# pixeru/bpm_analysis

Hardware: AMD Instinct MI355X
Metric: audio-samples/sec (filter+envelope+peaks), 1024x60s@44.1kHz batch, 1 & 8 GPU (higher is better)
Workload: dtype f64; 1 GPU; 1024 x 60 s 44100 Hz mono int16 recordings per GPU, native mode (filter+envelope+noise floor+raw peaks); mode=native, parallelism=file-sharded x1, batch_pipeline=False

## Files before the change

bpm_analysis_amd/_native.py:

```python
from __future__ import annotations

import ctypes
import os

_HERE = os.path.dirname(os.path.abspath(__file__))
LIB_PATH = os.environ.get("BPMX_LIB") or os.path.join(_HERE, "libbpmx.so")

ABI_VERSION = 2

DT_U8, DT_I16, DT_I32, DT_F32, DT_F64 = 0, 1, 2, 3, 4
MODE_REFERENCE, MODE_NATIVE = 0, 1
STAGE_ENVELOPE, STAGE_FLOOR, STAGE_PEAKS, STAGE_ALL = 1, 2, 4, 7
F_STATIC_FLOOR, F_DRAFT_FLOOR, F_NAN_FLOOR, F_TOO_SHORT, F_BAD_WINDOW = 1, 2, 4, 8, 16
F_TROUGH_TIE, F_PEAK_TIE = 32, 64
F_TROUGH_ORDERED, F_PEAK_ORDERED = 128, 256
OPT_ROLLQ_MERGE = 1
OPT_NATIVE_F64 = 2
OPT_HILBERT_ROCFFT = 4
OPT_DRAFT_FULL = 8
OPT_ROLLQ_NOPRUNE = 16
OPT_DRAFT_GLOBAL_RANK = 32
OPT_ROLLQ_GLOBAL = 64
OPT_NATIVE_DMA = 128
OPT_PEAKS_GLOBAL = 256
OPT_HILBERT_R2C = 512
OPT_REF_SERIAL_MEAN = 1024
OPT_STATS = 2048
OPT_HILBERT_BLUESTEIN = 4096
OPT_REF_NOSPLIT = 8192
STAT_RAW_TROUGHS, STAT_UNDECIDED, STAT_FULL_DRAFT, NSTATS = 0, 1, 2, 8
OK, E_ARG, E_HIP, E_LIMIT, E_NODEV = 0, -1, -2, -3, -4

EXPORTS = ["bpmx_abi_version", "bpmx_last_error", "bpmx_create", "bpmx_destroy", "bpmx_decimated_length",
           "bpmx_run", "bpmx_run_ordered", "bpmx_synth", "bpmx_synth_host", "bpmx_profile", "bpmx_profile_read", "bpmx_profile_only",
           "bpmx_stats", "bpmx_set_pipeline"]


class Params(ctypes.Structure):
    _fields_ = [("mode", ctypes.c_int32), ("stages", ctypes.c_int32), ("dtype", ctypes.c_int32),
                ("channels", ctypes.c_int32), ("fs", ctypes.c_int32), ("ds", ctypes.c_int32),
                ("sr", ctypes.c_int32), ("env_window", ctypes.c_int32), ("distance", ctypes.c_int32),
                ("noise_window", ctypes.c_int32), ("min_periods", ctypes.c_int32), ("options", ctypes.c_int32),
                ("trough_prom_q", ctypes.c_double), ("peak_prom_q", ctypes.c_double),
                ("noise_floor_q", ctypes.c_double), ("fallback_q", ctypes.c_double),
                ("reject_mult", ctypes.c_double),
                ("ba_b", ctypes.c_double * 5), ("ba_a", ctypes.c_double * 5), ("ba_zi", ctypes.c_double * 4),
                ("sos", ctypes.c_double * 12), ("sos_zi", ctypes.c_double * 4)]


class Batch(ctypes.Structure):
    _fields_ = [("n_files", ctypes.c_int32), ("reserved", ctypes.c_int32), ("pcm", ctypes.c_void_p),
                ("frame_offsets", ctypes.POINTER(ctypes.c_int64))]


class Out(ctypes.Structure):
    _fields_ = [("env", ctypes.c_void_p), ("floor", ctypes.c_void_p), ("y", ctypes.c_void_p),
                ("troughs", ctypes.c_void_p), ("peaks", ctypes.c_void_p), ("n_troughs", ctypes.c_void_p),
                ("n_peaks", ctypes.c_void_p), ("flags", ctypes.c_void_p), ("n_raw_troughs", ctypes.c_void_p)]


class PeakOrder(ctypes.Structure):
    _fields_ = [("cand", ctypes.c_void_p * 2), ("n_cand", ctypes.c_void_p * 2),
                ("rank", ctypes.c_void_p * 2), ("use_rank", ctypes.c_void_p * 2)]


class BpmxError(RuntimeError):

    def __init__(self, msg: str = "", code: int = None):
        super().__init__(msg)
        self.code = code

    @property
    def per_file(self) -> bool:
        return self.code in (E_ARG, E_LIMIT)


class BpmxArgError(BpmxError, ValueError):
    """BPMX_E_ARG: an argument the reference's own calls reject with ValueError
    (scipy find_peaks' distance check, pandas' rolling-window checks); the
    message is the library's, which repeats the reference-side wording."""


_lib = None
# ... 51 lines not shown
```

bpm_analysis_amd/csrc/bpmx_api.hip:

```cpp
#include <hip/hip_runtime.h>

#include <algorithm>
#include <climits>
#include <cstdio>
#include <cstring>
#include <cstdlib>
#include <map>
#include <mutex>
#include <string>
#include <vector>

#include "bpmx_common.h"
#include "bpmx_kernels.h"
#include "bpmx_ctx.h"
#include "bpmx_native.h"
#include "bpmx_fpscan.h"
#include "bpmx_synth.h"

#include <rocprofiler-sdk-roctx/roctx.h>

using namespace bpmx;

namespace bpmx {
thread_local std::string g_err;
// ... 622 lines not shown
            FIND_PEAKS(a, "troughs");
        }
        if (bad_window)
            LAUNCH(ctx, s, "k_flag_window", k_flag_window, dim3((F + 255) / 256), dim3(256), 0, s, F, d_run1,
                   (int32_t *)O->flags);
        const bool floor_wm = !(P->options & (BPMX_OPT_ROLLQ_MERGE | BPMX_OPT_ROLLQ_GLOBAL | BPMX_OPT_ROLLQ_NOPRUNE)) &&
                              maxnd <= WM_MMAX;
        if (noise_lazy && !floor_wm) {
            QuantArgs a;
            a.env = O->env; a.doff = d_doff; a.active = d_active; a.n_files = F; a.qv = qv; a.skip_le = QR_MAX;
            a.n_levels = 1; a.q[0] = P->noise_floor_q; a.slot[0] = 1 << Q_NOISE;
            a.skip = d_run1; a.stats = 0;
            LAUNCH(ctx, s, "k_quantile_reg", k_quantile_reg, dim3(F), dim3(QR_T), 0, s, a, bs);
        }
        const int64_t W = bad_window ? P->min_periods : P->noise_window;
        const int cap = (int)((W + RQ_T - 1 + 63) / 64 * 64);
        const size_t lds = rollq_lds_bytes(RQ_T, cap);
        const bool use_wm = !(P->options & (BPMX_OPT_ROLLQ_MERGE | BPMX_OPT_ROLLQ_GLOBAL));
        const bool need_merge = !use_wm || maxnd > WM_MMAX;
        const bool merge_g = need_merge && (cap > 32 * RQ_T || W + RQ_T >= 65000 || (P->options & BPMX_OPT_ROLLQ_GLOBAL));
        const int64_t gcap = (std::min<int64_t>(W + RQ_T, maxnd + 64) + 63) / 64 * 64;
        const size_t lds_g = rollq_g_lds_bytes(RQ_T, gcap);
        if (merge_g && lds_g > 160 * 1024)
            return fail(BPMX_E_LIMIT, "noise window and recording both longer than " +
                                          std::to_string((160 * 1024 - 16384) / 4 * 64) + " samples");
        uint16_t *wm_pos = use_wm ? (uint16_t *)ctx->buf("wm_pos", (size_t)sumnd * 2, &rc) : nullptr;
        int32_t *wm_full = use_wm ? (int32_t *)ctx->buf("wm_full", (size_t)F * 4, &rc) : nullptr;
        if (rc != BPMX_OK) return rc;
        const int64_t wm_n = std::min<int64_t>(maxnd, WM_MMAX);
        const size_t wm_lds_p = wm_layout(wm_n, true).total, wm_lds = wm_layout(wm_n, false).total;
        const int64_t wm_c = (WM_MMAX - W + 1) / 64 * 64;
        const bool wm_chunks = use_wm && maxnd > WM_MMAX && !(P->options & BPMX_OPT_ROLLQ_NOPRUNE) && wm_c >= 2048;
        const int64_t wm_nch = wm_chunks ? (maxnd + wm_c - 1) / wm_c : 1;
        int32_t *wm_fail = wm_chunks ? (int32_t *)ctx->buf("wm_fail", (size_t)F * 4, &rc) : nullptr;
        uint16_t *wm_pos_ch = wm_chunks ? (uint16_t *)ctx->buf("wm_pos_ch", (size_t)F * wm_nch * WM_PMAX * 2, &rc) : nullptr;
        if (rc != BPMX_OK) return rc;
        if (wm_nch > 65535) return fail(BPMX_E_LIMIT, "recording too long for the chunked rolling quantile");
        const dim3 g2((unsigned)std::min<int64_t>((maxnd + 255) / 256, std::max<int64_t>(8, 2048 / F)), F);
        auto interp = [&](const int32_t *run, const int64_t *tr, const int32_t *ntr, int64_t skip_gt) -> int {
            InterpArgs a;
            a.env = O->env; a.doff = d_doff; a.troughs = tr; a.ntr = ntr; a.run = run; a.n_files = F;
            a.dense = dense; a.skip_n = use_wm ? WM_MMAX : -1; a.skip_gt = skip_gt;
            const dim3 gi = maxnd <= WM_MMAX && use_wm ? dim3(2, (unsigned)F) : g2;
            LAUNCH(ctx, s, "k_interp", k_interp, gi, dim3(256), 0, s, a);
            return BPMX_OK;
        };
        auto rollq = [&](const int32_t *run, const int64_t *tr, const int32_t *ntr, double *outp,
                         int32_t *allnan, const double *tv) -> int {
            RollqArgs a;
            a.dense = dense; a.doff = d_doff; a.troughs = tr; a.tv = tv; a.run = run; a.n_files = F;
            a.env = O->env; a.ntr = ntr;
            a.window = (int32_t)W; a.min_periods = P->min_periods; a.cap = cap; a.q = P->noise_floor_q;
            a.out = outp; a.allnan = allnan; a.wm_max = use_wm ? WM_MMAX : 0;
            a.wm_chunk = 0; a.wm_fail = wm_fail; a.wm_pos_ch = wm_pos_ch;
            int rq_rc = BPMX_OK;
            int32_t *vfl = need_merge ? (int32_t *)ctx->buf("rollq_valid", (size_t)F * 8, &rq_rc) : nullptr;
            if (rq_rc != BPMX_OK) return rq_rc;
            a.vfirst = vfl;
            a.vlast = vfl ? vfl + F : nullptr;
            if (need_merge) {
                HIP_TRY(hipMemsetAsync(a.vfirst, 0x7F, (size_t)F * 4, s));
                HIP_TRY(hipMemsetAsync(a.vlast, 0xFF, (size_t)F * 4, s));
            }
            if (wm_chunks) {
                HIP_TRY(hipMemsetAsync(wm_fail, 0, (size_t)F * 4, s));
                a.wm_chunk = (int32_t)wm_c;
            }
            if (need_merge && (rq_rc = interp(run, tr, ntr, wm_chunks ? WM_MMAX : INT64_MAX)) != BPMX_OK) return rq_rc;
            if (use_wm) {
                wm_lds_attr(ctx->device);
                if (!(P->options & BPMX_OPT_ROLLQ_NOPRUNE))
                    LAUNCH(ctx, s, "k_rollq_wm", k_rollq_wm_t<true>, dim3(F, (unsigned)wm_nch), dim3(WM_T),
                           std::max(wm_lds_p, wm_lds), s, a, wm_pos, wm_full);
                else
                    LAUNCH(ctx, s, "k_rollq_wm[full]", k_rollq_wm_t<false>, dim3(F), dim3(WM_T), wm_lds, s, a, wm_pos,
                           wm_full);
            }
            if (!need_merge) return BPMX_OK;
            RollqArgs fill = a;
            if (wm_chunks) {
                a.run = wm_fail;
                if ((rq_rc = interp(wm_fail, tr, ntr, INT64_MAX)) != BPMX_OK) return rq_rc;
            }
            a.chunk = 8192;
            while (a.chunk > 1024 && (int64_t)F * ((maxnd + a.chunk - 1) / a.chunk) < 1024) a.chunk >>= 1;
            if (merge_g) a.chunk = std::max<int64_t>(a.chunk, (W + RQ_T - 1) / RQ_T * RQ_T);
            const int64_t nch = (maxnd + a.chunk - 1) / a.chunk;
            if (nch > 65535) return fail(BPMX_E_LIMIT, "recording too long for the chunked rolling quantile");
            const dim3 gq((unsigned)F, (unsigned)nch);
            if (merge_g) {
                a.gcap = gcap;
                a.gv = (double *)ctx->buf("rollq_gv", (size_t)F * nch * 2 * gcap * 8, &rq_rc);
                a.gp = (int32_t *)ctx->buf("rollq_gp", (size_t)F * nch * 2 * gcap * 4, &rq_rc);
                if (rq_rc != BPMX_OK) return rq_rc;
                (void)hipFuncSetAttribute((const void *)k_rolling_quantile_g<RQ_T>,
                                          hipFuncAttributeMaxDynamicSharedMemorySize, (int)lds_g);
                LAUNCH(ctx, s, "k_rolling_quantile", (k_rolling_quantile_g<RQ_T>), gq, dim3(RQ_T), lds_g, s, a);
            } else if (cap <= 16 * RQ_T) {
                (void)hipFuncSetAttribute((const void *)k_rolling_quantile<RQ_T, 16>,
                                          hipFuncAttributeMaxDynamicSharedMemorySize, (int)lds);
                LAUNCH(ctx, s, "k_rolling_quantile", (k_rolling_quantile<RQ_T, 16>), gq, dim3(RQ_T), lds, s, a);
            } else {
                (void)hipFuncSetAttribute((const void *)k_rolling_quantile<RQ_T, 32>,
                                          hipFuncAttributeMaxDynamicSharedMemorySize, (int)lds);
                LAUNCH(ctx, s, "k_rolling_quantile", (k_rolling_quantile<RQ_T, 32>), gq, dim3(RQ_T), lds, s, a);
            }
            LAUNCH(ctx, s, "k_rollq_fill", k_rollq_fill, dim3(4, (unsigned)F), dim3(256), 0, s, fill);
            return BPMX_OK;
        };
        uint8_t *tdec = nullptr;
        int32_t *d_exact = d_run1, *d_runfb = nullptr;
        if (bounds) {
            tdec = (uint8_t *)ctx->buf("trough_dec", (size_t)sumnd, &rc);
            if (rc != BPMX_OK) return rc;
            d_exact = draft_masks;
            d_runfb = draft_masks + F;
            DraftBoundArgs a;
            a.env = O->env; a.doff = d_doff; a.raw = rawt; a.rawv = rawv; a.nraw = d_nraw; a.run = d_run1;
            a.n_files = F;
            a.window = (int32_t)W; a.min_periods = P->min_periods; a.q = P->noise_floor_q; a.mult = P->reject_mult;
            a.dec = tdec; a.exact = d_exact;
            a.local_m = (P->options & BPMX_OPT_DRAFT_GLOBAL_RANK) ? INT_MAX : DB_LOCAL_M;
            a.stats = d_stats;
            if (rc != BPMX_OK) return rc;
            const int64_t trmax = maxnd / std::max<int64_t>(1, P->distance) + 1;
            const unsigned gy = (unsigned)std::max<int64_t>(1, (trmax + DB_T - 1) / DB_T);
            a.vfl = draft_vfl;
            a.nund = draft_vfl + 2 * F;
            LAUNCH(ctx, s, "k_draft_bounds", k_draft_bounds, dim3(F, gy), dim3(DB_T), 0, s, a);
#ifndef BPMX_DP_GY
#define BPMX_DP_GY 4
#endif
            const unsigned gp = (unsigned)std::max<int64_t>(1, std::min<int64_t>(BPMX_DP_GY, (trmax + DP_CHUNK - 1) / DP_CHUNK));
            LAUNCH(ctx, s, "k_draft_points", k_draft_points<1>, dim3(F, gp), dim3(DB_T), 0, s, a);
            LAUNCH(ctx, s, "k_draft_points[wide]", k_draft_points<4>, dim3(F, gp), dim3(DB_T), 0, s, a);
        }
        SanitizeArgs sa;
        sa.env = O->env; sa.draft = draft; sa.doff = d_doff; sa.active = d_active; sa.raw = rawt; sa.nraw = d_nraw;
        sa.rawv = rawv; sa.outv = trv;
        sa.n_files = F; sa.mult = P->reject_mult; sa.out = O->troughs; sa.nout = O->n_troughs; sa.flags = O->flags;
        sa.run2 = d_run2; sa.dec = tdec; sa.exact = d_exact; sa.run_fb = d_runfb;
        if (floor_wm) {
            FloorWmArgs a;
            a.rq.dense = dense; a.rq.doff = d_doff; a.rq.n_files = F; a.rq.env = O->env;
            a.rq.window = (int32_t)W; a.rq.min_periods = P->min_periods; a.rq.cap = cap; a.rq.q = P->noise_floor_q;
            a.rq.wm_max = WM_MMAX; a.rq.wm_chunk = 0; a.rq.wm_fail = nullptr; a.rq.wm_pos_ch = nullptr;
            a.rq.vfirst = a.rq.vlast = nullptr; a.rq.chunk = 0; a.rq.gv = nullptr; a.rq.gp = nullptr; a.rq.gcap = 0;
            a.rq.troughs = nullptr; a.rq.tv = nullptr; a.rq.ntr = nullptr; a.rq.run = nullptr; a.rq.out = nullptr;
            a.rq.allnan = nullptr;
#ifdef BPMX_STAMPS
            a.rq.stamps = nullptr;
#endif
            sa.run2 = nullptr; sa.run_fb = nullptr;
            a.sa = sa;
            a.exact = d_exact;
            a.qv = qv;
            a.qn = QuantArgs{};
            if (noise_lazy) {
                a.qn.env = O->env; a.qn.doff = d_doff; a.qn.active = d_active; a.qn.n_files = F; a.qn.qv = qv;
                a.qn.skip_le = QR_MAX; a.qn.n_levels = 1; a.qn.q[0] = P->noise_floor_q; a.qn.slot[0] = 1 << Q_NOISE;
                a.qn.skip = nullptr; a.qn.stats = 0;
            }
            a.floor = O->floor; a.draft = draft; a.an_draft = d_an1; a.an_final = d_an2; a.full = wm_full;
            if ((rc = rollq(d_exact, rawt, d_nraw, draft, d_an1, rawv)) != BPMX_OK) return rc;
            wm_lds_attr(ctx->device);
            LAUNCH(ctx, s, "k_floor_wm", k_floor_wm, dim3(F), dim3(WM_T), std::max(wm_lds_p, wm_lds), s, a);
        }
        if (!floor_wm && (rc = rollq(d_exact, rawt, d_nraw, draft, d_an1, rawv)) != BPMX_OK) return rc;
        if (!floor_wm) {
            SanitizeArgs a;
            a.env = O->env; a.draft = draft; a.doff = d_doff; a.active = d_active; a.raw = rawt; a.nraw = d_nraw;
            a.rawv = rawv; a.outv = trv;
            a.n_files = F; a.mult = P->reject_mult; a.out = O->troughs; a.nout = O->n_troughs; a.flags = O->flags;
            a.run2 = d_run2; a.dec = tdec; a.exact = d_exact; a.run_fb = d_runfb;
            LAUNCH(ctx, s, "k_sanitize", k_sanitize, dim3(F), dim3(256), 0, s, a);
        }
        if (!floor_wm && bounds && (rc = rollq(d_runfb, rawt, d_nraw, draft, d_an1, rawv)) != BPMX_OK) return rc;
        if (!floor_wm && (rc = rollq(d_run2, O->troughs, O->n_troughs, O->floor, d_an2, trv)) != BPMX_OK) return rc;
        if (!floor_wm) {
            FinalArgs a;
            a.draft = draft; a.doff = d_doff; a.active = d_active; a.qv = qv; a.allnan_draft = d_an1;
            a.allnan_final = d_an2; a.n_files = F; a.floor = O->floor; a.flags = O->flags;
#ifndef BPMX_FF_WIDE
            const dim3 gf(maxnd > 65536 ? g2.x : 1u, (unsigned)F);
#else
            const dim3 gf = g2;
#endif
            LAUNCH(ctx, s, "k_floor_final", k_floor_final, gf, dim3(256), 0, s, a);
        }
    }

    if (do_peaks) {
        StageRange range("bpmx:peaks");
        PeakArgs a;
        a.env = O->env; a.height = O->floor; a.doff = d_doff; a.boff = d_boff; a.active = d_active;
        a.bmax = bmax; a.bmin = bmin; a.qv = qv; a.qslot = Q_PEAK; a.n_files = F; a.distance = P->distance;
        a.sign = 1.0; a.cand = cand; a.state = state; a.out = O->peaks; a.nout = O->n_peaks;
        a.run_out = nullptr; a.run_min = 0; a.tie_bit = BPMX_F_PEAK_TIE;
        a.scan_ok = fp_scan; a.scan_cnt = fp_scan + F;
        set_order(a, 1);
        FIND_PEAKS(a, "peaks");
    }
// ... 161 lines not shown
```

bpm_analysis_amd/csrc/bpmx_kernels.h:

```cpp
#ifndef BPMX_KERNELS_H
#define BPMX_KERNELS_H

#include "bpmx_common.h"

namespace bpmx {

enum { Q_TROUGH = 0, Q_PEAK = 1, Q_NOISE = 2, Q_FALLBACK = 3, Q_SLOTS = 4 };

struct InitOutArgs {
    const int32_t *active;
    int32_t *flags, *ntr, *npk, *runs, *nraw;
    int32_t *z1;
    int32_t *z2;
    int32_t *z3;
    int32_t n_files;
};
__device__ __forceinline__ void init_out_one(const InitOutArgs &I, int f) {
    const int F = I.n_files;
    I.flags[f] = I.active[f] ? 0 : BPMX_F_TOO_SHORT;
    if (I.ntr) I.ntr[f] = 0;
    if (I.npk) I.npk[f] = 0;
    for (int k = 0; k < 5; ++k) I.runs[(int64_t)k * F + f] = 0;
    if (I.nraw) I.nraw[f] = 0;
    if (I.z1) I.z1[f] = 0;
// ... 159 lines not shown
    int32_t *mtot;
    int32_t *mp;
    double *mh;
    double *vv;
    double *b32h, *b32l, *b32r;
    double *b1kh, *b1kl, *b1kr;
    int32_t *dfail;
    int32_t dchunk;
};
constexpr int FPC_T = 256, FPC_S = 1024, FPC_H = 1024, FPC_R = (FPC_S + FPC_H) / FPC_T;
__host__ __device__ inline int64_t fpl_b32_off(int64_t d0, int f) { return (d0 >> 5) + 4 * (int64_t)f; }
__host__ __device__ inline int64_t fpl_b1k_off(int64_t d0, int f) { return (d0 >> 10) + 4 * (int64_t)f; }
__global__ void k_fpl_scan(PeakArgs A, FplArgs L);
__global__ void k_fpl_place(PeakArgs A, FplArgs L);
__global__ void k_fpl_fill(PeakArgs A, FplArgs L);
__global__ void k_fpl_distance(PeakArgs A, FplArgs L);
__global__ void k_fpl_dist_ch(PeakArgs A, FplArgs L);
__global__ void k_fpl_prom(PeakArgs A, FplArgs L);
__global__ void k_fpl_compact(PeakArgs A, FplArgs L);

struct InterpArgs {
    const double *env;
    const int64_t *doff;
    const int64_t *troughs;
    const int32_t *ntr;
    const int32_t *run;
    int32_t n_files;
    double *dense;
    int64_t skip_n;
    int64_t skip_gt;
};

struct RollqArgs {
    const double *dense;
    const int64_t *doff;
    const int64_t *troughs;
    const int32_t *run;
    int32_t n_files, window, min_periods, cap;
    double q;
    double *out;
    int32_t *allnan;
    int32_t wm_max;
    const double *env;
    const double *tv;
    const int32_t *ntr;
    int64_t chunk;
    int32_t *vfirst, *vlast;
    double *gv;
    int32_t *gp;
    int64_t gcap;
    int32_t wm_chunk;
    int32_t *wm_fail;
    uint16_t *wm_pos_ch;
#ifdef BPMX_STAMPS
    unsigned long long *stamps;
#endif
};

struct SanitizeArgs {
    const double *env, *draft;
    const int64_t *doff;
    const int32_t *active;
    const int64_t *raw;
    const double *rawv;
    const int32_t *nraw;
    int32_t n_files;
    double mult;
    double *outv;
    int64_t *out;
    int32_t *nout;
    int32_t *flags;
    int32_t *run2;
    const uint8_t *dec;
    const int32_t *exact;
    int32_t *run_fb;
};

template <int NT>
__device__ __forceinline__ int sanitize_wg(const SanitizeArgs &A, int f, int *sh) {
    const int64_t d0 = A.doff[f];
    const int64_t *raw = A.raw + d0;
    int64_t *out = A.out + d0;
    const int m = A.nraw[f];
    const int tid = threadIdx.x;
    const double *rawv = A.rawv + d0;
    double *outv = A.outv + d0;
    if (m < 5) {
        for (int j = tid; j < m; j += NT) { out[j] = raw[j]; outv[j] = rawv[j]; }
        if (tid == 0) {
            A.nout[f] = m;
            A.flags[f] |= BPMX_F_STATIC_FLOOR;
            if (A.run2) A.run2[f] = 0;
        }
        return m;
    }
    const double *draft = A.draft + d0;
    const bool exact = !A.dec || A.exact[f];
    int w = 0;
    for (int c0 = 0; c0 < m; c0 += NT) {
        const int j = c0 + tid;
        bool keep = false;
        int64_t t = 0;
        double tv = 0.0;
        if (j < m) {
            t = raw[j];
            tv = rawv[j];
// ... 49 lines not shown
constexpr int DB_T = 256;
constexpr int DB_TRMAX = 2040;
constexpr int DB_LOCAL_M = 512;
struct DbSeg {
    int32_t s, e;
    double v;
};

struct FinalArgs {
    const double *draft;
    const int64_t *doff;
    const int32_t *active;
    const double *qv;
    const int32_t *allnan_draft, *allnan_final;
    int32_t n_files;
    double *floor;
    int32_t *flags;
};

__host__ __device__ inline size_t rollq_lds_bytes(int T, int cap) {
    return (size_t)cap * 10 + (size_t)T * 20 + ((size_t)T + 1) * 4 + ((size_t)T / 64 + 2) * 4;
}
constexpr int RQ_T = 256;

template <int DT, bool MULTI, bool ZB>
__global__ void k_envelope_ref_t(EnvRefArgs A);
template <int DT, bool MULTI>
__global__ void k_ref_pick(EnvRefArgs A);
__global__ void k_quantile_reg(QuantArgs A, BlockStatArgs B);
__global__ void k_block_stats(BlockStatArgs A);
__global__ void k_find_peaks(PeakArgs A);
__global__ void k_find_peaks_lds(PeakArgs A);
__global__ void k_interp(InterpArgs A);
__global__ void k_sanitize(SanitizeArgs A);
__global__ void k_draft_bounds(DraftBoundArgs A);
template <int SPL>
__global__ void k_draft_points(DraftBoundArgs A);
__global__ void k_floor_final(FinalArgs A);
template <int T, int RQ_MAXCH>
__global__ void k_rolling_quantile(RollqArgs A);
template <int T>
__global__ void k_rolling_quantile_g(RollqArgs A);
__host__ __device__ inline size_t rollq_g_lds_bytes(int T, int64_t gcap) {
    return (size_t)T * 16 + (size_t)T * 8 + ((size_t)T + 1) * 4 + ((size_t)T / 64 + 2) * 4 + (size_t)T * 16 +
           ((size_t)(gcap / 64) + 2) * 4;
}
__global__ void k_rollq_fill(RollqArgs A);

constexpr int WM_T = 1024;
constexpr int WM_ITEMS = 18;
constexpr int WM_MMAX = WM_T * WM_ITEMS;
constexpr int WM_TRMAX = 512;
constexpr int WM_PMAX = 12288;
constexpr int WM_DCAP = 96;
constexpr int WM_WSCR = WM_DCAP;
struct WmLayout {
    size_t tab, meta, kpos, area, total;
};
constexpr int WM_NBK = WM_MMAX / 64 + 2;
constexpr int WM_META_LOW = (WM_NBK * 22 + 7) & ~7;
constexpr int WM_META_B = WM_META_LOW + WM_NBK * 22;
__host__ __device__ inline size_t wm_align16(size_t x) { return (x + 15) & ~(size_t)15; }
__host__ __device__ inline WmLayout wm_layout(int64_t nmax, bool prune) {
    const int64_t n = nmax < 1 ? 1 : (nmax > WM_MMAX ? WM_MMAX : nmax);
    const int64_t m = prune && n > WM_PMAX ? WM_PMAX : n;
    const int64_t L = m > 1 ? 64 - __builtin_clzll((unsigned long long)(m - 1)) : 1;
    const int64_t NW = (m + 63) / 64;
    const int64_t m8 = (m + 7) & ~7LL;
    const int64_t NBK = WM_MMAX / 64 + 2;
    const int64_t sort_b = 8 * m8 + (int64_t)(WM_T / 64) * 128 * 4;
    const int64_t wm_b = ((4 * m8 + 15) & ~15LL) + (int64_t)(WM_T / 64) * WM_WSCR * 4;
    (void)L; (void)NW;
    const int64_t hist_b = prune ? NBK * 64 * 2 + (int64_t)(WM_T / 64) * 64 * 4 + n : 0;
    int64_t area = sort_b > wm_b ? sort_b : wm_b;
    area = area > hist_b ? area : hist_b;
    WmLayout l;
    l.tab = 0;
    l.meta = wm_align16((size_t)WM_TRMAX * (prune ? 20 : 12) + (size_t)NBK * 4);
    l.kpos = wm_align16(l.meta + (prune ? (size_t)WM_META_B : 0));
    l.area = wm_align16(l.kpos + (prune ? (size_t)m * 2 : 0));
    l.total = l.area + (size_t)area;
    return l;
}
template <bool PRUNE>
__global__ void k_rollq_wm_t(RollqArgs A, uint16_t *pos_scratch, int32_t *full);
__global__ void k_floor_wm(FloorWmArgs A);

}

#endif
```

bpm_analysis_amd/csrc/k_rollq_wm.hip:

```cpp
#include "bpmx_common.h"
#include "bpmx_kernels.h"
#include "bpmx_stamps.h"
#include "bpmx_qsel.h"

namespace bpmx {

__device__ __forceinline__ uint64_t wm_key(double v) {
    return f64_key(v == 0.0 ? 0.0 : v);
}

__device__ __forceinline__ uint64_t lanemask_lt() {
    return (1ull << lane_id()) - 1ull;
}

__device__ __forceinline__ uint64_t match8(uint32_t dg) {
    uint64_t m = ~0ull;
#pragma unroll
    for (int b = 0; b < 8; ++b) {
        const uint64_t bal = __ballot((dg >> b) & 1u);
        m &= ((dg >> b) & 1u) ? bal : ~bal;
    }
    return m;
}

// ... 309 lines not shown
            if (lane == 0) {
                pre[NPB] = run;
                if (!wid) s_mk = run;
            }
        }
        __syncthreads();
        kc = s_mk;
        STAMP(13);
        if (kc > WM_PMAX) {
            if (tid == 0) { if (chunked) A.wm_fail[f] = 1; else full[f] = 1; }
            return !chunked;
        }
        if (tid == 0 && !chunked) full[f] = 0;
        for (int pb = wid; pb < NPB; pb += NWV) {
            const uint64_t mk = kmask[pb];
            if ((mk >> lane) & 1) kpos[kpre[pb] + __popcll(mk & lanemask_lt())] = (uint16_t)((pb << 6) + lane);
        }
        m = kc;
        __syncthreads();
    }
#ifdef RQ_STOP_PRUNE
    return false;
#endif
    auto spos = [&](int c) -> int { return PRUNE ? (int)kpos[c] : c; };
    auto kidx = [&](int p) -> int {
        if (!PRUNE) return p;
        const uint64_t mk = kmask[p >> 6];
        return kpre[p >> 6] + __popcll(mk & ((1ull << (p & 63)) - 1ull));
    };
    auto lidx = [&](int p) -> int {
        const uint64_t mk = lmask[p >> 6];
        return lpre[p >> 6] + __popcll(mk & ((1ull << (p & 63)) - 1ull));
    };
    STAMP(7);
#ifdef RQ_DIAG_M
    if (threadIdx.x == 0) _st_acc[13] = (unsigned long long)m;
#endif

    const int IT = (m + WM_T - 1) / WM_T;
    const int mu = __builtin_amdgcn_readfirstlane(m), ITu = __builtin_amdgcn_readfirstlane(IT);
    const int S = 64 * IT;
    const int m8 = (m + 7) & ~7;
    uint16_t *posA = (uint16_t *)(smem + Lay.area);
    uint16_t *posB = posA + m8;
    uint32_t *kh = (uint32_t *)(posB + m8);
    uint32_t *cnt = kh + m8;
    const size_t wbin_off = (size_t)8 * m8 + (size_t)NWV * 128 * 4;
    unsigned long long *wbin_all =
        wbin_off + (size_t)NWV * 256 * 8 <= Lay.total - Lay.area ? (unsigned long long *)(smem + Lay.area + wbin_off) : nullptr;

    const size_t wsc = ((size_t)4 * m8 + 15) & ~(size_t)15;
    const size_t svl_off = wsc + (size_t)NWV * WM_WSCR * 4;
    double *svl = svl_off + (size_t)8 * m <= Lay.total - Lay.area ? (double *)(smem + Lay.area + svl_off) : nullptr;
    uint64_t kbase = 0;
    int shc = 0;
    if (PRUNE && svl) {
        kbase = wm_key(s_vmin);
        const uint64_t ktop = wm_key(s_vmax);
        const int nbits = ktop > kbase ? 64 - __clzll((long long)(ktop - kbase)) : 0;
        shc = nbits > 40 ? nbits - 40 : 0;
    }
    {
        auto ckey = [&](int p) -> uint64_t {
            const uint64_t k = wm_key(dval(t0 + spos(p)));
            return shc ? (k > kbase ? k - kbase : 0ull) >> shc : k;
        };
        uint64_t kor = 0, kand = ~0ull;
        for (int p = tid; p < m; p += WM_T) {
            posA[p] = (uint16_t)p;
            const uint64_t k = ckey(p);
            kh[p] = (uint32_t)k;
            kor |= k;
            kand &= k;
        }
        for (int o = 32; o > 0; o >>= 1) {
            kor |= (uint64_t)__shfl_xor((long long)kor, o);
            kand &= (uint64_t)__shfl_xor((long long)kand, o);
        }
        if (lane == 0) { s_or[wid] = kor; s_and[wid] = kand; }
        if (wbin_all)
            for (int j = tid; j < NWV * 256; j += WM_T) wbin_all[j] = 0ull;
        __syncthreads();
        uint64_t vary = 0;
        {
            uint64_t o = 0, a = ~0ull;
            for (int w = 0; w < NWV; ++w) { o |= s_or[w]; a &= s_and[w]; }
            vary = o ^ a;
        }
        STAMP(0);
        uint32_t *wc = cnt + wid * 128;
        for (int d = 0; d < 8; ++d) {
            if (d == 4 && (vary >> 32)) {
                for (int p = tid; p < m; p += WM_T) kh[p] = (uint32_t)(ckey(p) >> 32);
                __syncthreads();
            }
            if (((vary >> (8 * d)) & 0xFFull) == 0) continue;
            const int sh = 8 * (d & 3);
            for (int j = lane; j < 128; j += 64) wc[j] = 0;
            uint32_t dg8[(MAXIT + 3) / 4], rk16[(MAXIT + 1) / 2];
            int mo = mu, ITo = ITu, sb = wid * S + lane;
            asm volatile("" : "+s"(mo), "+s"(ITo), "+v"(sb));
#pragma unroll
            for (int i = 0; i < MAXIT; ++i) {
                const int slot = sb + i * 64;
                const uint32_t dg = (i < ITo && slot < mo) ? (kh[posA[slot]] >> sh) & 0xFFu : 0u;
                if ((i & 3) == 0) dg8[i >> 2] = dg; else dg8[i >> 2] |= dg << (8 * (i & 3));
            }
            __builtin_amdgcn_wave_barrier();
            asm volatile("" : "+s"(mo), "+s"(ITo), "+v"(sb));
#pragma unroll
            for (int i = 0; i < MAXIT; ++i) {
                if (i < ITo) {
                    const int slot = sb + i * 64;
                    const bool valid = slot < mo;
                    const uint32_t dg = (dg8[i >> 2] >> (8 * (i & 3))) & 0xFFu;
                    uint64_t peers;
                    if (wbin_all) {
                        unsigned long long *bin = wbin_all + wid * 256 + dg;
                        if (valid) atomicOr(bin, 1ull << lane);
                        peers = __hip_atomic_load(bin, __ATOMIC_RELAXED, __HIP_MEMORY_SCOPE_WORKGROUP);
                    } else {
                        peers = match8(dg);
                    }
                    peers &= __ballot(valid);
                    const uint64_t below = peers & lanemask_lt();
                    const int leader = valid ? __ffsll((long long)peers) - 1 : lane;
                    uint32_t base = 0;
                    if (valid && below == 0) {
                        base = atomicAdd(&wc[dg >> 1], (uint32_t)__popcll(peers) << (16 * (dg & 1)));
                        if (wbin_all) __hip_atomic_store(wbin_all + wid * 256 + dg, 0ull, __ATOMIC_RELAXED,
                                                         __HIP_MEMORY_SCOPE_WORKGROUP);
                    }
                    base = (uint32_t)__shfl((int)base, leader);
                    const uint32_t rnk = ((base >> (16 * (dg & 1))) & 0xFFFFu) + (uint32_t)__popcll(below);
                    if ((i & 1) == 0) rk16[i >> 1] = rnk; else rk16[i >> 1] |= rnk << 16;
// ... 3 lines not shown
            STAMP(1);
            {
                uint32_t v[4], sm = 0;
#pragma unroll
                for (int u = 0; u < 4; ++u) {
                    const int e = tid * 4 + u, dg = e / NWV, w = e % NWV;
                    v[u] = (cnt[w * 128 + (dg >> 1)] >> (16 * (dg & 1))) & 0xFFFFu;
                    sm += v[u];
                }
                uint32_t x = sm;
                for (int o = 1; o < 64; o <<= 1) {
                    const uint32_t y = __shfl_up(x, o);
                    if (lane >= o) x += y;
                }
                if (lane == 63) s_wt[wid] = (int)x;
                __syncthreads();
                uint32_t run = x - sm;
                for (int w = 0; w < wid; ++w) run += (uint32_t)s_wt[w];
                uint16_t *c16 = (uint16_t *)cnt;
#pragma unroll
                for (int u = 0; u < 4; ++u) {
                    const int e = tid * 4 + u, dg = e / NWV, w = e % NWV;
                    c16[(w * 128 + (dg >> 1)) * 2 + (dg & 1)] = (uint16_t)run;
                    run += v[u];
                }
            }
            __syncthreads();
            STAMP(2);
            const uint16_t *c16 = (const uint16_t *)cnt;
            asm volatile("" : "+s"(mo), "+s"(ITo), "+v"(sb));
#pragma unroll
            for (int i = 0; i < MAXIT; ++i) {
                const int slot = sb + i * 64;
                if (i < ITo && slot < mo) {
                    const uint32_t dg = (dg8[i >> 2] >> (8 * (i & 3))) & 0xFFu;
                    const uint32_t rnk = (rk16[i >> 1] >> (16 * (i & 1))) & 0xFFFFu;
                    posB[(int)c16[(wid * 128 + (dg >> 1)) * 2 + (dg & 1)] + (int)rnk] = posA[slot];
                }
            }
            __syncthreads();
            uint16_t *t = posA; posA = posB; posB = t;
            STAMP(3);
        }
    }
    uint16_t *posR = posA, *rkx = posB;
    for (int r = tid; r < m; r += WM_T) rkx[posR[r]] = (uint16_t)r;
    if (svl)
        for (int r = tid; r < m; r += WM_T) svl[r] = dval(t0 + spos(posR[r]));
    __syncthreads();
    if (shc) {
        bool down = false;
        for (int r = tid; r + 1 < m; r += WM_T) down |= svl[r] > svl[r + 1];
        if (__syncthreads_or(down)) {
            if (tid == 0) { if (chunked) A.wm_fail[f] = 1; else full[f] = 1; }
            return !chunked;
        }
    }
#ifdef RQ_STOP_SORT
    return false;
#endif
    uint32_t *wl = (uint32_t *)(smem + Lay.area + wsc) + (size_t)wid * WM_WSCR;
    STAMP(5);

    auto target = [&](int nb, double &idxf, bool &interp) -> int {
        idxf = 0;
        int k = 0;
        if (nb > 1) {
            idxf = q * (double)(nb - 1);
            k = (int)idxf;
        }
        interp = !(nb == 1 || (double)k == idxf);
        return k;
    };
    const uint64_t ltm = lanemask_lt();
    const int off = (int)((W - 1) / 2), Wi = (int)W, ni = (int)n, t0i = (int)t0;
#ifdef RQ_DIAG_Q
    unsigned long long dq[8] = {0};
#endif
    int vfirst = INT_MAX, vlast = -1;
#ifdef RQ_DIAG_W
    const unsigned long long tw0 = __builtin_amdgcn_s_memtime();
#endif
    {
        const int NBLK = (int)((o1 - o0 + 63) >> 6);
        const int NBW = (NBLK + NWV - 1) / NWV;
        const int b0 = wid * NBW, b1 = min(NBLK, b0 + NBW);
        int rs = 0, cU = 0, pPlo = -1, pPhi = -1;
        for (int bk = b0; bk < b1; ++bk) {
            const int i0 = (int)o0 + (bk << 6), i = i0 + lane;
            bool valid = false;
            int plo = 0, phi = 0, t = 0, nobs = 0, kq = 0;
            double idxq = 0.0;
            bool intq = false;
            if (i < (int)o1) {
                const int ee = i + 1 + off, ss = ee - Wi;
                const int e = ee < ni ? ee : ni, sc = ss > 0 ? ss : 0;
                const int lo = sc > t0i ? sc : t0i;
                nobs = e > lo ? e - lo : 0;
                if (nobs >= minp && nobs > 0) {
                    valid = true;
                    plo = kidx(lo - t0i);
                    phi = kidx(e - t0i);
                    const int lw = PRUNE ? lidx(e - t0i) - lidx(lo - t0i) : 0;
                    kq = target(nobs, idxq, intq);
                    t = kq - lw;
                }
            }
            const uint64_t vm0 = __ballot(valid);
// ... 286 lines not shown
```

bpm_analysis_amd/engine.py:

```python
from __future__ import annotations

import ctypes
import threading
from dataclasses import dataclass
from typing import List, Optional, Sequence

import numpy as np

from . import _native as N
from .design import Design, design, detect_design, dtype_code, make_params

MODES = {"reference": N.MODE_REFERENCE, "native": N.MODE_NATIVE}


def _torch():
    import torch
    return torch


_TORCH_DT = None


def torch_dtype(np_dtype):
    global _TORCH_DT
# ... 222 lines not shown
        ev = torch.cuda.Event()
        ev.record(torch.cuda.current_stream(self.device))
        return host, ev

    def tie_check_finish(self, handle, out: Result, params: dict, stages: int = N.STAGE_ALL,
                         options: int = 0) -> int:
        host, ev = handle
        ev.synchronize()
        bits = N.F_TROUGH_TIE | N.F_PEAK_TIE
        if not (host.numpy() & bits).any():
            return 0
        return self.resolve_ties(out, params, stages, options)

    def synth(self, frame_offsets: Sequence[int], fs: int, channels: int = 1, seed0: int = 0,
              seeds: Optional[Sequence[int]] = None):
        torch = _torch()
        fo = np.ascontiguousarray(frame_offsets, dtype=np.int64)
        pcm = torch.empty(int(fo[-1]) * channels, dtype=torch.int16, device=self.device)
        runs = [(seed0, 0, len(fo) - 1)] if seeds is None else [(int(sd), f, f + 1) for f, sd in enumerate(seeds)]
        with self.lock:
            for sd, a, b in runs:
                sub = np.ascontiguousarray(fo[a:b + 1])
                N.check(self.L.bpmx_synth(self.ctx, sd, b - a, sub.ctypes.data_as(ctypes.POINTER(ctypes.c_int64)),
                                          fs, channels, ctypes.c_void_p(pcm.data_ptr()), self.stream_handle()),
                        "bpmx_synth")
        return pcm

    def profile(self, on: bool):
        N.check(self.L.bpmx_profile(self.ctx, 1 if on else 0), "bpmx_profile")

    def profile_only(self, label: str = ""):
        N.check(self.L.bpmx_profile_only(self.ctx, label.encode()), "bpmx_profile_only")

    def profile_read(self) -> dict:
        buf = ctypes.create_string_buffer(1 << 16)
        n = self.L.bpmx_profile_read(self.ctx, buf, len(buf))
        if n < 0:
            N.check(n, "bpmx_profile_read")
        out = {}
        for line in buf.value.decode().splitlines():
            name, cnt, ms = line.rsplit(" ", 2)
            out[name] = (int(cnt), float(ms))
        return out

    def set_pipeline(self, chunks: int, env_cus: int = 0, det_cus: int = 0):
        N.check(self.L.bpmx_set_pipeline(self.ctx, chunks, env_cus, det_cus), "bpmx_set_pipeline")

    def stats(self) -> dict:
        buf = (ctypes.c_int64 * N.NSTATS)()
        rc = self.L.bpmx_stats(self.ctx, buf, N.NSTATS)
        if rc < 0:
            N.check(rc, "bpmx_stats")
        return {"raw_troughs": int(buf[N.STAT_RAW_TROUGHS]), "undecided": int(buf[N.STAT_UNDECIDED]),
                "full_draft_chunks": int(buf[N.STAT_FULL_DRAFT])}

    def run_host(self, recordings: List[np.ndarray], fs: int, params: dict, mode: str = "reference",
                 stages: int = N.STAGE_ALL, want_y: bool = False, log: bool = False,
                 options: int = 0, longest_first: bool = True, resolve_ties: bool = False) -> List[dict]:
        torch = _torch()
        if not recordings:
            return []
        if longest_first and len({r.shape[0] for r in recordings}) > 1:
            from .shard import longest_first as _lf
            perm = _lf([r.shape[0] for r in recordings])
            res = self.run_host([recordings[i] for i in perm], fs, params, mode=mode, stages=stages,
                                want_y=want_y, log=log, options=options, longest_first=False,
                                resolve_ties=resolve_ties)
            out: List[dict] = [None] * len(recordings)
            for k, i in enumerate(perm):
                out[i] = res[k]
            return out
        dt = recordings[0].dtype
        ch = 1 if recordings[0].ndim == 1 else recordings[0].shape[1]
        for r in recordings:
            if r.dtype != dt or (1 if r.ndim == 1 else r.shape[1]) != ch:
                raise ValueError("a batch needs one sample format and channel count")
        fo = np.zeros(len(recordings) + 1, dtype=np.int64)
        fo[1:] = np.cumsum([r.shape[0] for r in recordings])
        host = np.concatenate([np.ascontiguousarray(r).reshape(-1) for r in recordings])
        with self.lock, torch.cuda.stream(self.host_stream()):
            pcm = torch.from_numpy(host).to(self.device)
            res = self.run(pcm, fo, fs, params, mode=mode, stages=stages, channels=ch, want_y=want_y, log=log,
                           options=options)
            if resolve_ties:
                self.resolve_ties(res, params, stages, options)
            out = res.to_host()
            self.host_stream().synchronize()
        return out

    def run_env_host(self, envs: List[np.ndarray], sr: int, params: dict, stages: int,
                     floors: Optional[List[np.ndarray]] = None, options: int = 0,
                     resolve_ties: bool = False) -> List[dict]:
        torch = _torch()
        fo = np.zeros(len(envs) + 1, dtype=np.int64)
        fo[1:] = np.cumsum([len(e) for e in envs])
        d = detect_design(sr, params)
        with self.lock, torch.cuda.stream(self.host_stream()):
            out = self.alloc(fo, 1, d.sr)
            out.env.copy_(torch.from_numpy(np.concatenate(envs).astype(np.float64)).to(self.device))
            if floors is not None:
                out.floor.copy_(torch.from_numpy(np.concatenate(floors).astype(np.float64)).to(self.device))
            self.run(None, fo, d.sr, params, stages=stages, out=out, d=d, options=options)
            if resolve_ties:
                self.resolve_ties(out, params, stages, options)
            res = out.to_host()
            self.host_stream().synchronize()
        return res
# ... 127 lines not shown
```

include/bpmx.h:

```cpp
#ifndef BPMX_H
#define BPMX_H

#include <stdint.h>

#ifdef __cplusplus
extern "C" {
#endif

#define BPMX_ABI_VERSION 2

enum bpmx_dtype { BPMX_DT_U8 = 0, BPMX_DT_I16 = 1, BPMX_DT_I32 = 2, BPMX_DT_F32 = 3, BPMX_DT_F64 = 4 };

enum bpmx_mode { BPMX_MODE_REFERENCE = 0, BPMX_MODE_NATIVE = 1 };

enum bpmx_stage {
    BPMX_STAGE_ENVELOPE = 1,
    BPMX_STAGE_FLOOR = 2,
    BPMX_STAGE_PEAKS = 4,
    BPMX_STAGE_ALL = 7
};

enum bpmx_status {
    BPMX_OK = 0,
    BPMX_E_ARG = -1,
    BPMX_E_HIP = -2,
    BPMX_E_LIMIT = -3,
    BPMX_E_NODEV = -4
};

enum bpmx_file_flag {
    BPMX_F_STATIC_FLOOR = 1,
    BPMX_F_DRAFT_FLOOR = 2,
    BPMX_F_NAN_FLOOR = 4,
    BPMX_F_TOO_SHORT = 8,
    BPMX_F_BAD_WINDOW = 16,
    BPMX_F_TROUGH_TIE = 32,
    BPMX_F_PEAK_TIE = 64,
    BPMX_F_TROUGH_ORDERED = 128,
    BPMX_F_PEAK_ORDERED = 256
};

enum bpmx_option {
    BPMX_OPT_ROLLQ_MERGE = 1,
    BPMX_OPT_NATIVE_F64 = 2,
    BPMX_OPT_HILBERT_ROCFFT = 4,
    BPMX_OPT_DRAFT_FULL = 8,
    BPMX_OPT_ROLLQ_NOPRUNE = 16,
    BPMX_OPT_DRAFT_GLOBAL_RANK = 32,
    BPMX_OPT_ROLLQ_GLOBAL = 64,
    BPMX_OPT_NATIVE_DMA = 128,
    BPMX_OPT_PEAKS_GLOBAL = 256,
    BPMX_OPT_HILBERT_R2C = 512,
    BPMX_OPT_REF_SERIAL_MEAN = 1024,
    BPMX_OPT_STATS = 2048,
    BPMX_OPT_HILBERT_BLUESTEIN = 4096,
    BPMX_OPT_REF_NOSPLIT = 8192
};

enum bpmx_stat {
    BPMX_STAT_RAW_TROUGHS = 0,
    BPMX_STAT_UNDECIDED = 1,
    BPMX_STAT_FULL_DRAFT = 2,
    BPMX_NSTATS = 8
};

typedef struct bpmx_ctx bpmx_ctx;

typedef struct {
    int32_t mode;
    int32_t stages;
    int32_t dtype;
    int32_t channels;
    int32_t fs;
    int32_t ds;
    int32_t sr;
    int32_t env_window;
    int32_t distance;
    int32_t noise_window;
    int32_t min_periods;
    int32_t options;
    double trough_prom_q;
    double peak_prom_q;
    double noise_floor_q;
    double fallback_q;
    double reject_mult;
    double ba_b[5], ba_a[5], ba_zi[4];
    double sos[12], sos_zi[4];
} bpmx_params;

typedef struct {
    int32_t n_files;
    int32_t reserved;
    const void *pcm;
    const int64_t *frame_offsets;
} bpmx_batch;

typedef struct {
    double *env;
    double *floor;
    double *y;
    int64_t *troughs;
    int64_t *peaks;
    int32_t *n_troughs;
    int32_t *n_peaks;
    int32_t *flags;
    int32_t *n_raw_troughs;
} bpmx_out;

int bpmx_abi_version(void);
const char *bpmx_last_error(void);

int bpmx_create(int device, bpmx_ctx **out);
void bpmx_destroy(bpmx_ctx *ctx);

int64_t bpmx_decimated_length(int64_t n_frames, int32_t ds);
// ... 32 lines not shown
```

Baseline: 1158 billion audio-samples/s.

## Repair near-sorted rank order in-kernel instead of falling back to full redo

In the wavelet-matrix rolling quantile kernel, a detected out-of-order sorted value list previously marked the file or chunk as failed and forced a slower fallback path. It now runs up to a few odd-even transposition passes to fix local inversions and rebuilds the rank index, falling back only if the order is still broken. Key compaction now stashes keys in shared memory, computes the exact min/max with a block reduction, and shifts down to 32 significant bits instead of 40. Stats counters for repair passes and redos are added. The price is extra shared memory, extra barriers and some sorting work.

```diff
diff --git a/bpm_analysis_amd/_native.py b/bpm_analysis_amd/_native.py
--- a/bpm_analysis_amd/_native.py
+++ b/bpm_analysis_amd/_native.py
@@ -29,6 +29,7 @@
 OPT_HILBERT_BLUESTEIN = 4096
 OPT_REF_NOSPLIT = 8192
 STAT_RAW_TROUGHS, STAT_UNDECIDED, STAT_FULL_DRAFT, NSTATS = 0, 1, 2, 8
+STAT_RANK_REDO, STAT_RANK_REPAIR = 3, 4
 OK, E_ARG, E_HIP, E_LIMIT, E_NODEV = 0, -1, -2, -3, -4
 
 EXPORTS = ["bpmx_abi_version", "bpmx_last_error", "bpmx_create", "bpmx_destroy", "bpmx_decimated_length",
diff --git a/bpm_analysis_amd/csrc/bpmx_api.hip b/bpm_analysis_amd/csrc/bpmx_api.hip
--- a/bpm_analysis_amd/csrc/bpmx_api.hip
+++ b/bpm_analysis_amd/csrc/bpmx_api.hip
@@ -698,7 +698,7 @@
             a.env = O->env; a.ntr = ntr;
             a.window = (int32_t)W; a.min_periods = P->min_periods; a.cap = cap; a.q = P->noise_floor_q;
             a.out = outp; a.allnan = allnan; a.wm_max = use_wm ? WM_MMAX : 0;
-            a.wm_chunk = 0; a.wm_fail = wm_fail; a.wm_pos_ch = wm_pos_ch;
+            a.wm_chunk = 0; a.wm_fail = wm_fail; a.wm_pos_ch = wm_pos_ch; a.stats = d_stats;
             int rq_rc = BPMX_OK;
             int32_t *vfl = need_merge ? (int32_t *)ctx->buf("rollq_valid", (size_t)F * 8, &rq_rc) : nullptr;
             if (rq_rc != BPMX_OK) return rq_rc;
@@ -793,7 +793,7 @@
             a.rq.wm_max = WM_MMAX; a.rq.wm_chunk = 0; a.rq.wm_fail = nullptr; a.rq.wm_pos_ch = nullptr;
             a.rq.vfirst = a.rq.vlast = nullptr; a.rq.chunk = 0; a.rq.gv = nullptr; a.rq.gp = nullptr; a.rq.gcap = 0;
             a.rq.troughs = nullptr; a.rq.tv = nullptr; a.rq.ntr = nullptr; a.rq.run = nullptr; a.rq.out = nullptr;
-            a.rq.allnan = nullptr;
+            a.rq.allnan = nullptr; a.rq.stats = d_stats;
 #ifdef BPMX_STAMPS
             a.rq.stamps = nullptr;
 #endif
diff --git a/bpm_analysis_amd/csrc/bpmx_kernels.h b/bpm_analysis_amd/csrc/bpmx_kernels.h
--- a/bpm_analysis_amd/csrc/bpmx_kernels.h
+++ b/bpm_analysis_amd/csrc/bpmx_kernels.h
@@ -235,6 +235,7 @@
     int32_t wm_chunk;
     int32_t *wm_fail;
     uint16_t *wm_pos_ch;
+    int64_t *stats;
 #ifdef BPMX_STAMPS
     unsigned long long *stamps;
 #endif
@@ -390,6 +391,7 @@
 constexpr int WM_MMAX = WM_T * WM_ITEMS;
 constexpr int WM_TRMAX = 512;
 constexpr int WM_PMAX = 12288;
+constexpr int WM_REPAIR = 4;
 constexpr int WM_DCAP = 96;
 constexpr int WM_WSCR = WM_DCAP;
 struct WmLayout {
diff --git a/bpm_analysis_amd/csrc/k_rollq_wm.hip b/bpm_analysis_amd/csrc/k_rollq_wm.hip
--- a/bpm_analysis_amd/csrc/k_rollq_wm.hip
+++ b/bpm_analysis_amd/csrc/k_rollq_wm.hip
@@ -385,18 +385,39 @@
     const size_t wsc = ((size_t)4 * m8 + 15) & ~(size_t)15;
     const size_t svl_off = wsc + (size_t)NWV * WM_WSCR * 4;
     double *svl = svl_off + (size_t)8 * m <= Lay.total - Lay.area ? (double *)(smem + Lay.area + svl_off) : nullptr;
+    const bool compact = PRUNE && svl != nullptr && (size_t)16 * m8 + (size_t)NWV * 16 <= Lay.total - Lay.area;
+    uint64_t *stash = (uint64_t *)(smem + Lay.area + (size_t)8 * m8);
+    uint64_t *s_klo = stash + m8, *s_khi = s_klo + NWV;
     uint64_t kbase = 0;
     int shc = 0;
-    if (PRUNE && svl) {
-        kbase = wm_key(s_vmin);
-        const uint64_t ktop = wm_key(s_vmax);
-        const int nbits = ktop > kbase ? 64 - __clzll((long long)(ktop - kbase)) : 0;
-        shc = nbits > 40 ? nbits - 40 : 0;
+    if (compact) {
+        uint64_t lo = ~0ull, hi = 0ull;
+        for (int p = tid; p < m; p += WM_T) {
+            const uint64_t k = wm_key(dval(t0 + spos(p)));
+            stash[p] = k;
+            lo = k < lo ? k : lo;
+            hi = k > hi ? k : hi;
+        }
+        for (int o = 32; o > 0; o >>= 1) {
+            const uint64_t xl = (uint64_t)__shfl_xor((long long)lo, o), xh = (uint64_t)__shfl_xor((long long)hi, o);
+            lo = xl < lo ? xl : lo;
+            hi = xh > hi ? xh : hi;
+        }
+        if (lane == 0) { s_klo[wid] = lo; s_khi[wid] = hi; }
+        __syncthreads();
+        for (int w = 0; w < NWV; ++w) {
+            const uint64_t xl = s_klo[w], xh = s_khi[w];
+            lo = xl < lo ? xl : lo;
+            hi = xh > hi ? xh : hi;
+        }
+        kbase = lo;
+        const int nbits = hi > lo ? 64 - __clzll((long long)(hi - lo)) : 0;
+        shc = nbits > 32 ? nbits - 32 : 0;
     }
     {
         auto ckey = [&](int p) -> uint64_t {
-            const uint64_t k = wm_key(dval(t0 + spos(p)));
-            return shc ? (k > kbase ? k - kbase : 0ull) >> shc : k;
+            if (compact) return (stash[p] - kbase) >> shc;
+            return wm_key(dval(t0 + spos(p)));
         };
         uint64_t kor = 0, kand = ~0ull;
         for (int p = tid; p < m; p += WM_T) {
@@ -411,9 +432,9 @@
             kand &= (uint64_t)__shfl_xor((long long)kand, o);
         }
         if (lane == 0) { s_or[wid] = kor; s_and[wid] = kand; }
+        __syncthreads();
         if (wbin_all)
-            for (int j = tid; j < NWV * 256; j += WM_T) wbin_all[j] = 0ull;
-        __syncthreads();
+            for (int j = lane; j < 256; j += 64) wbin_all[wid * 256 + j] = 0ull;
         uint64_t vary = 0;
         {
             uint64_t o = 0, a = ~0ull;
@@ -523,8 +544,33 @@
         bool down = false;
         for (int r = tid; r + 1 < m; r += WM_T) down |= svl[r] > svl[r + 1];
         if (__syncthreads_or(down)) {
-            if (tid == 0) { if (chunked) A.wm_fail[f] = 1; else full[f] = 1; }
-            return !chunked;
+            int pass = 0;
+            do {
+                down = false;
+                for (int ph = 0; ph < 2; ++ph) {
+                    for (int r = 2 * tid + ph; r + 1 < m; r += 2 * WM_T) {
+                        const double a = svl[r], b = svl[r + 1];
+                        if (a > b) {
+                            const uint16_t pa = posR[r], pb = posR[r + 1];
+                            svl[r] = b; svl[r + 1] = a;
+                            posR[r] = pb; posR[r + 1] = pa;
+                            down = true;
+                        }
+                    }
+                    __syncthreads();
+                }
+                down = __syncthreads_or(down) != 0;
+            } while (down && ++pass <= WM_REPAIR);
+            if (A.stats && tid == 0) atomicAdd((unsigned long long *)&A.stats[BPMX_STAT_RANK_REPAIR], (unsigned long long)pass);
+            if (down) {
+                if (tid == 0) {
+                    if (A.stats) atomicAdd((unsigned long long *)&A.stats[BPMX_STAT_RANK_REDO], 1ull);
+                    if (chunked) A.wm_fail[f] = 1; else full[f] = 1;
+                }
+                return !chunked;
+            }
+            for (int r = tid; r < m; r += WM_T) rkx[posR[r]] = (uint16_t)r;
+            __syncthreads();
         }
     }
 #ifdef RQ_STOP_SORT
diff --git a/bpm_analysis_amd/engine.py b/bpm_analysis_amd/engine.py
--- a/bpm_analysis_amd/engine.py
+++ b/bpm_analysis_amd/engine.py
@@ -298,7 +298,8 @@
         if rc < 0:
             N.check(rc, "bpmx_stats")
         return {"raw_troughs": int(buf[N.STAT_RAW_TROUGHS]), "undecided": int(buf[N.STAT_UNDECIDED]),
-                "full_draft_chunks": int(buf[N.STAT_FULL_DRAFT])}
+                "full_draft_chunks": int(buf[N.STAT_FULL_DRAFT]),
+                "rank_redo": int(buf[N.STAT_RANK_REDO]), "rank_repair_passes": int(buf[N.STAT_RANK_REPAIR])}
 
     def run_host(self, recordings: List[np.ndarray], fs: int, params: dict, mode: str = "reference",
                  stages: int = N.STAGE_ALL, want_y: bool = False, log: bool = False,
diff --git a/include/bpmx.h b/include/bpmx.h
--- a/include/bpmx.h
+++ b/include/bpmx.h
@@ -61,6 +61,8 @@
     BPMX_STAT_RAW_TROUGHS = 0,
     BPMX_STAT_UNDECIDED = 1,
     BPMX_STAT_FULL_DRAFT = 2,
+    BPMX_STAT_RANK_REDO = 3,
+    BPMX_STAT_RANK_REPAIR = 4,
     BPMX_NSTATS = 8
 };
 
```

Result: faster. 1171 billion audio-samples/s, median of 6 (+1.1%).
